# ugadiarov-la-phystech-edu/OCRL

Measured on AMD Instinct MI355X. Metric: images/sec (node) SLATE pretrain 128x128, 6 slots, 3 iters, higher is better.
Workload: dtype f32

## Files before the change

ocrl_amd/csrc/attention.hip:

```cpp
#include "common.h"
#include "kernels.h"
#include <stdlib.h>

#define FA_BLK 64
#ifndef FA_LPT
#define FA_LPT 1
#endif
#ifndef FA_BWD_WGS
#define FA_BWD_WGS 3
#endif

typedef float f32x4_t __attribute__((ext_vector_type(4)));

template <int DH>
struct FaCfg {
    static constexpr int NC = DH / 16;
    static constexpr int LD = DH + 4;
};

template <int DH>
__device__ inline void fa_load_tile(float* s, const float* __restrict__ g, long long bt0, int row0, int T, int d, int hoff, float scale) {
    constexpr int F4 = DH / 4;
    constexpr int LD = FaCfg<DH>::LD;
    for (int idx = threadIdx.x; idx < FA_BLK * F4; idx += 256) {
        const int c4 = idx % F4, r = idx / F4;
        float4 v = make_float4(0.f, 0.f, 0.f, 0.f);
        if (row0 + r < T) v = *reinterpret_cast<const float4*>(g + (bt0 + row0 + r) * d + hoff + c4 * 4);
        v.x *= scale; v.y *= scale; v.z *= scale; v.w *= scale;
        *reinterpret_cast<float4*>(s + r * LD + c4 * 4) = v;
    }
}

template <int DH> struct FaRegs { static constexpr int N = (FA_BLK * (DH / 4) + 255) / 256; };
template <int DH>
__device__ inline void fa_fetch(float4 (&r)[FaRegs<DH>::N], const float* __restrict__ g, long long bt0, int row0, int T, int d, int hoff) {
    constexpr int F4 = DH / 4;
#pragma unroll
    for (int i = 0; i < FaRegs<DH>::N; ++i) {
        const int idx = threadIdx.x + i * 256;
        const int c4 = idx % F4, row = idx / F4;
        r[i] = make_float4(0.f, 0.f, 0.f, 0.f);
        if (idx < FA_BLK * F4 && row0 + row < T) r[i] = *reinterpret_cast<const float4*>(g + (bt0 + row0 + row) * d + hoff + c4 * 4);
    }
}
template <int DH>
__device__ inline void fa_commit(float* s, const float4 (&r)[FaRegs<DH>::N], float scale) {
    constexpr int F4 = DH / 4, LD = FaCfg<DH>::LD;
#pragma unroll
    for (int i = 0; i < FaRegs<DH>::N; ++i) {
        const int idx = threadIdx.x + i * 256;
        if (idx < FA_BLK * F4) *reinterpret_cast<float4*>(s + (idx / F4) * LD + (idx % F4) * 4) = make_float4(r[i].x * scale, r[i].y * scale, r[i].z * scale, r[i].w * scale);
    }
}

__device__ inline int fa_block_index(int j, long long bh, int nblk) {
    const long long rot = nblk >= 8 ? bh : bh / (8 / (nblk > 0 ? nblk : 1) > 0 ? 8 / nblk : 1);
    return (int)((j + rot) % nblk);
}

#define MFMA16(a, b, c) __builtin_amdgcn_mfma_f32_16x16x4f32((a), (b), (c), 0, 0, 0)

template <int DH>
__global__ __launch_bounds__(256, 4) void attn_fwd_kernel(AttnArgs p) {
    constexpr int NC = FaCfg<DH>::NC, LD = FaCfg<DH>::LD;
    __shared__ __attribute__((aligned(16))) float Ks[FA_BLK * LD];
    __shared__ __attribute__((aligned(16))) float Vs[FA_BLK * LD];
    const int nqb = (p.T + FA_BLK - 1) / FA_BLK;
    int bid = blockIdx.x;
    const int nbh = gridDim.x / nqb;
    const int qb = FA_LPT ? nqb - 1 - bid / nbh : fa_block_index(bid % nqb, bid / nqb, nqb);
    bid = FA_LPT ? bid % nbh : bid / nqb;
    const int hd = bid % p.h;
    const long long b = bid / p.h;
    const int T = p.T, d = p.ld, hoff = hd * DH;
    const long long bt0 = b * T;
    const int lane = threadIdx.x & 63, wv = threadIdx.x >> 6;
    const int li = lane & 15, g = lane >> 4;
    const int q_abs = qb * FA_BLK + wv * 16 + li;
    const float scale = rsqrtf((float)DH);
    const long long bh = b * p.h + hd;

    float4 qf[NC];
#pragma unroll
    for (int c = 0; c < NC; ++c) {
        float4 v = make_float4(0.f, 0.f, 0.f, 0.f);
        if (q_abs < T) v = *reinterpret_cast<const float4*>(p.q + (bt0 + q_abs) * d + hoff + 16 * c + 4 * g);
        qf[c] = make_float4(v.x * scale, v.y * scale, v.z * scale, v.w * scale);
    }
    f32x4_t o[NC];
#pragma unroll
    for (int c = 0; c < NC; ++c) o[c] = (f32x4_t){0.f, 0.f, 0.f, 0.f};
    float m = -INFINITY, l = 0.f;
    const uint32_t thr = drop_thresh(p.p);
    const float dsc = p.p > 0.f ? 1.0f / (1.0f - p.p) : 1.f;

    float4 rk[FaRegs<DH>::N], rv[FaRegs<DH>::N];
    fa_fetch<DH>(rk, p.k, bt0, 0, T, d, hoff);
    fa_fetch<DH>(rv, p.v, bt0, 0, T, d, hoff);
    for (int kt = 0; kt <= qb; ++kt) {
        __syncthreads();
        fa_commit<DH>(Ks, rk, 1.f);
        fa_commit<DH>(Vs, rv, 1.f);
        __syncthreads();
        if (kt < qb) {
            fa_fetch<DH>(rk, p.k, bt0, (kt + 1) * FA_BLK, T, d, hoff);
            fa_fetch<DH>(rv, p.v, bt0, (kt + 1) * FA_BLK, T, d, hoff);
        }
        f32x4_t s[4];
#pragma unroll
        for (int st = 0; st < 4; ++st) s[st] = (f32x4_t){0.f, 0.f, 0.f, 0.f};
#pragma unroll
        for (int c = 0; c < NC; ++c) {
            float4 a[4];
#pragma unroll
            for (int st = 0; st < 4; ++st) a[st] = *reinterpret_cast<const float4*>(Ks + (16 * st + li) * LD + 16 * c + 4 * g);
#pragma unroll
            for (int st = 0; st < 4; ++st) s[st] = MFMA16(a[st].x, qf[c].x, s[st]);
#pragma unroll
            for (int st = 0; st < 4; ++st) s[st] = MFMA16(a[st].y, qf[c].y, s[st]);
#pragma unroll
            for (int st = 0; st < 4; ++st) s[st] = MFMA16(a[st].z, qf[c].z, s[st]);
#pragma unroll
            for (int st = 0; st < 4; ++st) s[st] = MFMA16(a[st].w, qf[c].w, s[st]);
        }
        float mx = -INFINITY;
        if (kt == qb || (kt + 1) * FA_BLK > T) {
#pragma unroll
            for (int st = 0; st < 4; ++st) {
                const int key0 = kt * FA_BLK + 16 * st + 4 * g;
#pragma unroll
                for (int r = 0; r < 4; ++r)
                    if (key0 + r > q_abs || key0 + r >= T) s[st][r] = -INFINITY;
            }
        }
#pragma unroll
        for (int st = 0; st < 4; ++st)
#pragma unroll
            for (int r = 0; r < 4; ++r) mx = fmaxf(mx, s[st][r]);
        mx = fmaxf(mx, __shfl_xor(mx, 16, 64));
        mx = fmaxf(mx, __shfl_xor(mx, 32, 64));
        const float m_new = fmaxf(m, mx);
        const float alpha = (m_new == -INFINITY) ? 1.f : __expf(m - m_new);
        float rs = 0.f;
#pragma unroll
        for (int st = 0; st < 4; ++st)
#pragma unroll
            for (int r = 0; r < 4; ++r) {
                const float e = (m_new == -INFINITY) ? 0.f : __expf(s[st][r] - m_new);
                s[st][r] = e;
                rs += e;
            }
        rs += __shfl_xor(rs, 16, 64);
        rs += __shfl_xor(rs, 32, 64);
        l = l * alpha + rs;
        m = m_new;
#pragma unroll
        for (int c = 0; c < NC; ++c) o[c] *= alpha;
        if (p.p > 0.f) {
#pragma unroll
            for (int st = 0; st < 4; ++st) {
                const uint64_t idx = ((uint64_t)bh * T + (uint64_t)(q_abs < T ? q_abs : 0)) * T + (uint64_t)(kt * FA_BLK + 16 * st + 4 * g);
                const uint2 bits = rng_bits4(p.seed, p.site, idx >> 2);
#pragma unroll
                for (int r = 0; r < 4; ++r) s[st][r] = rng_keep(bits, r, thr) ? s[st][r] * dsc : 0.f;
            }
        }
        float av[2][4][NC];
#pragma unroll
        for (int r = 0; r < 4; ++r)
#pragma unroll
            for (int c = 0; c < NC; ++c) av[0][r][c] = Vs[(4 * g + r) * LD + 16 * c + li];
#pragma unroll
        for (int st = 0; st < 4; ++st) {
            if (st + 1 < 4) {
#pragma unroll
                for (int r = 0; r < 4; ++r)
#pragma unroll
                    for (int c = 0; c < NC; ++c) av[(st + 1) & 1][r][c] = Vs[(16 * (st + 1) + 4 * g + r) * LD + 16 * c + li];
            }
            __builtin_amdgcn_sched_barrier(0);
#pragma unroll
            for (int r = 0; r < 4; ++r)
#pragma unroll
                for (int c = 0; c < NC; ++c) o[c] = MFMA16(av[st & 1][r][c], s[st][r], o[c]);
            __builtin_amdgcn_sched_barrier(0);
        }
    }
    if (q_abs < T) {
        const float inv = 1.0f / l;
#pragma unroll
        for (int c = 0; c < NC; ++c)
            *reinterpret_cast<float4*>(p.o + (bt0 + q_abs) * p.d + hoff + 16 * c + 4 * g) = make_float4(o[c][0] * inv, o[c][1] * inv, o[c][2] * inv, o[c][3] * inv);
        if (g == 0) p.lse[bh * T + q_abs] = m + __logf(l);
    }
}

__global__ __launch_bounds__(256) void attn_delta_kernel(const float* __restrict__ dO, const float* __restrict__ O, float* __restrict__ delta, long long BT, int T, int d,
                                                         int h) {
    __shared__ float part[256];
    const int F4 = d >> 2, RPB = 256 / F4, HF = F4 / h;
    const int rl = threadIdx.x / F4, c4 = threadIdx.x - rl * F4;
    const long long row = (long long)blockIdx.x * RPB + rl;
    float s = 0.f;
    if (rl < RPB && row < BT) {
        const float4 x = *reinterpret_cast<const float4*>(dO + row * d + c4 * 4), y = *reinterpret_cast<const float4*>(O + row * d + c4 * 4);
        s = x.x * y.x + x.y * y.y + x.z * y.z + x.w * y.w;
    }
    part[threadIdx.x] = s;
    __syncthreads();
    if ((int)threadIdx.x < RPB * h) {
        const int r2 = threadIdx.x / h, hd = threadIdx.x - r2 * h;
        const long long row2 = (long long)blockIdx.x * RPB + r2;
        if (row2 < BT) {
            float t = 0.f;
            for (int k = 0; k < HF; ++k) t += part[r2 * F4 + hd * HF + k];
            const long long bb = row2 / T, q = row2 % T;
            delta[(bb * h + hd) * T + q] = t;
        }
    }
}

template <int DH>
__global__ __launch_bounds__(256, FA_BWD_WGS) void attn_bwd_kv_kernel(AttnArgs p) {
    constexpr int NC = FaCfg<DH>::NC, LD = FaCfg<DH>::LD;
    __shared__ __attribute__((aligned(16))) float Qs[FA_BLK * LD];
    __shared__ __attribute__((aligned(16))) float Gs[FA_BLK * LD];
    __shared__ float Ls[FA_BLK], Ds[FA_BLK];
    const int nkb = (p.T + FA_BLK - 1) / FA_BLK;
    int bid = blockIdx.x;
    const int nbh = gridDim.x / nkb;
    const int kb = FA_LPT ? bid / nbh : fa_block_index(bid % nkb, bid / nkb, nkb);
    bid = FA_LPT ? bid % nbh : bid / nkb;
    const int hd = bid % p.h;
    const long long b = bid / p.h;
    const int T = p.T, d = p.ld, hoff = hd * DH;
    const long long bt0 = b * T;
    const int lane = threadIdx.x & 63, wv = threadIdx.x >> 6;
    const int li = lane & 15, g = lane >> 4;
    const int k_abs = kb * FA_BLK + wv * 16 + li;
    const float scale = rsqrtf((float)DH);
    const long long bh = b * p.h + hd;

    float4 kf[NC], vf[NC];
#pragma unroll
    for (int c = 0; c < NC; ++c) {
        kf[c] = make_float4(0.f, 0.f, 0.f, 0.f);
        vf[c] = kf[c];
        if (k_abs < T) {
            kf[c] = *reinterpret_cast<const float4*>(p.k + (bt0 + k_abs) * d + hoff + 16 * c + 4 * g);
            vf[c] = *reinterpret_cast<const float4*>(p.v + (bt0 + k_abs) * d + hoff + 16 * c + 4 * g);
        }
    }
    f32x4_t dk[NC], dv[NC];
#pragma unroll
    for (int c = 0; c < NC; ++c) { dk[c] = (f32x4_t){0.f, 0.f, 0.f, 0.f}; dv[c] = dk[c]; }
    const uint32_t thr = drop_thresh(p.p);
    const float dsc = p.p > 0.f ? 1.0f / (1.0f - p.p) : 1.f;

    float4 rq[FaRegs<DH>::N], rg[FaRegs<DH>::N];
    float rl = 0.f, rd = 0.f;
    auto fetch = [&](int qt) {
        fa_fetch<DH>(rq, p.q, bt0, qt * FA_BLK, T, d, hoff);
        fa_fetch<DH>(rg, p.dO, bt0, qt * FA_BLK, T, p.d, hoff);
        if (threadIdx.x < FA_BLK) {
            const int qq = qt * FA_BLK + threadIdx.x;
            rl = qq < T ? p.lse[bh * T + qq] : 0.f;
            rd = qq < T ? p.delta[bh * T + qq] : 0.f;
        }
    };
    fetch(kb);
    for (int qt = kb; qt < nkb; ++qt) {
        __syncthreads();
        fa_commit<DH>(Qs, rq, scale);
        fa_commit<DH>(Gs, rg, 1.f);
        if (threadIdx.x < FA_BLK) { Ls[threadIdx.x] = rl; Ds[threadIdx.x] = rd; }
        __syncthreads();
        if (qt + 1 < nkb) fetch(qt + 1);
#pragma unroll
        for (int sq = 0; sq < 4; ++sq) {
            f32x4_t s = (f32x4_t){0.f, 0.f, 0.f, 0.f}, dp = s;
#pragma unroll
            for (int c = 0; c < NC; ++c) {
                const float4 a = *reinterpret_cast<const float4*>(Qs + (16 * sq + li) * LD + 16 * c + 4 * g);
                s = MFMA16(a.x, kf[c].x, s);
                s = MFMA16(a.y, kf[c].y, s);
                s = MFMA16(a.z, kf[c].z, s);
                s = MFMA16(a.w, kf[c].w, s);
                const float4 e = *reinterpret_cast<const float4*>(Gs + (16 * sq + li) * LD + 16 * c + 4 * g);
                dp = MFMA16(e.x, vf[c].x, dp);
                dp = MFMA16(e.y, vf[c].y, dp);
                dp = MFMA16(e.z, vf[c].z, dp);
                dp = MFMA16(e.w, vf[c].w, dp);
            }
            uint2 hb = make_uint2(0u, 0u);
            if (p.p > 0.f) {
                const int qh = qt * FA_BLK + 16 * sq + 4 * g + (li & 3);
                const uint64_t idx = ((uint64_t)bh * T + (uint64_t)(qh < T ? qh : 0)) * T + (uint64_t)(k_abs < T ? k_abs : 0);
                hb = rng_bits4(p.seed, p.site, idx >> 2);
            }
            uint2 hq[4];
            hq[0] = make_uint2(__builtin_amdgcn_update_dpp(0, (int)hb.x, 0x00, 0xF, 0xF, false), __builtin_amdgcn_update_dpp(0, (int)hb.y, 0x00, 0xF, 0xF, false));
            hq[1] = make_uint2(__builtin_amdgcn_update_dpp(0, (int)hb.x, 0x55, 0xF, 0xF, false), __builtin_amdgcn_update_dpp(0, (int)hb.y, 0x55, 0xF, 0xF, false));
            hq[2] = make_uint2(__builtin_amdgcn_update_dpp(0, (int)hb.x, 0xAA, 0xF, 0xF, false), __builtin_amdgcn_update_dpp(0, (int)hb.y, 0xAA, 0xF, 0xF, false));
            hq[3] = make_uint2(__builtin_amdgcn_update_dpp(0, (int)hb.x, 0xFF, 0xF, 0xF, false), __builtin_amdgcn_update_dpp(0, (int)hb.y, 0xFF, 0xF, 0xF, false));
            f32x4_t pd, ds;
#pragma unroll
            for (int r = 0; r < 4; ++r) {
                const int ql = 16 * sq + 4 * g + r;
                const int qa = qt * FA_BLK + ql;
                float pr = 0.f;
                if (qa < T && k_abs <= qa && k_abs < T) pr = __expf(s[r] - Ls[ql]);
                float keep = 1.f;
                if (p.p > 0.f) keep = rng_keep(hq[r], li & 3, thr) ? dsc : 0.f;
                pd[r] = pr * keep;
                ds[r] = pr * (dp[r] * keep - Ds[ql]);
            }
            float ag[4][NC], aq[4][NC];
#pragma unroll
            for (int r = 0; r < 4; ++r)
#pragma unroll
                for (int c = 0; c < NC; ++c) {
                    ag[r][c] = Gs[(16 * sq + 4 * g + r) * LD + 16 * c + li];
                    aq[r][c] = Qs[(16 * sq + 4 * g + r) * LD + 16 * c + li];
                }
            __builtin_amdgcn_sched_barrier(0);
#pragma unroll
            for (int r = 0; r < 4; ++r)
#pragma unroll
                for (int c = 0; c < NC; ++c) {
                    dv[c] = MFMA16(ag[r][c], pd[r], dv[c]);
                    dk[c] = MFMA16(aq[r][c], ds[r], dk[c]);
                }
        }
    }
    if (k_abs < T) {
#pragma unroll
        for (int c = 0; c < NC; ++c) {
            *reinterpret_cast<float4*>(p.dv + (bt0 + k_abs) * d + hoff + 16 * c + 4 * g) = make_float4(dv[c][0], dv[c][1], dv[c][2], dv[c][3]);
            *reinterpret_cast<float4*>(p.dk + (bt0 + k_abs) * d + hoff + 16 * c + 4 * g) = make_float4(dk[c][0], dk[c][1], dk[c][2], dk[c][3]);
        }
    }
}

template <int DH>
__global__ __launch_bounds__(256, FA_BWD_WGS) void attn_bwd_q_kernel(AttnArgs p) {
    constexpr int NC = FaCfg<DH>::NC, LD = FaCfg<DH>::LD;
    __shared__ __attribute__((aligned(16))) float Ks[FA_BLK * LD];
    __shared__ __attribute__((aligned(16))) float Vs[FA_BLK * LD];
    const int nqb = (p.T + FA_BLK - 1) / FA_BLK;
    int bid = blockIdx.x;
    const int nbh = gridDim.x / nqb;
    const int qb = FA_LPT ? nqb - 1 - bid / nbh : fa_block_index(bid % nqb, bid / nqb, nqb);
    bid = FA_LPT ? bid % nbh : bid / nqb;
    const int hd = bid % p.h;
    const long long b = bid / p.h;
    const int T = p.T, d = p.ld, hoff = hd * DH;
    const long long bt0 = b * T;
    const int lane = threadIdx.x & 63, wv = threadIdx.x >> 6;
    const int li = lane & 15, g = lane >> 4;
    const int q_abs = qb * FA_BLK + wv * 16 + li;
    const float scale = rsqrtf((float)DH);
    const long long bh = b * p.h + hd;

    float4 qf[NC], gf[NC];
#pragma unroll
    for (int c = 0; c < NC; ++c) {
        qf[c] = make_float4(0.f, 0.f, 0.f, 0.f);
        gf[c] = qf[c];
        if (q_abs < T) {
            const float4 v = *reinterpret_cast<const float4*>(p.q + (bt0 + q_abs) * d + hoff + 16 * c + 4 * g);
            qf[c] = make_float4(v.x * scale, v.y * scale, v.z * scale, v.w * scale);
            gf[c] = *reinterpret_cast<const float4*>(p.dO + (bt0 + q_abs) * p.d + hoff + 16 * c + 4 * g);
        }
    }
    const float lse = q_abs < T ? p.lse[bh * T + q_abs] : 0.f;
    const float dlt = q_abs < T ? p.delta[bh * T + q_abs] : 0.f;
    f32x4_t dq[NC];
#pragma unroll
    for (int c = 0; c < NC; ++c) dq[c] = (f32x4_t){0.f, 0.f, 0.f, 0.f};
    const uint32_t thr = drop_thresh(p.p);
    const float dsc = p.p > 0.f ? 1.0f / (1.0f - p.p) : 1.f;

    float4 rk[FaRegs<DH>::N], rv[FaRegs<DH>::N];
    fa_fetch<DH>(rk, p.k, bt0, 0, T, d, hoff);
    fa_fetch<DH>(rv, p.v, bt0, 0, T, d, hoff);
    for (int kt = 0; kt <= qb; ++kt) {
        __syncthreads();
        fa_commit<DH>(Ks, rk, 1.f);
        fa_commit<DH>(Vs, rv, 1.f);
        __syncthreads();
        if (kt < qb) {
            fa_fetch<DH>(rk, p.k, bt0, (kt + 1) * FA_BLK, T, d, hoff);
            fa_fetch<DH>(rv, p.v, bt0, (kt + 1) * FA_BLK, T, d, hoff);
        }
        f32x4_t sS[4], sP[4];
#pragma unroll
        for (int st = 0; st < 4; ++st) { sS[st] = (f32x4_t){0.f, 0.f, 0.f, 0.f}; sP[st] = sS[st]; }
#pragma unroll
        for (int c = 0; c < NC; ++c) {
            float4 a[4], e[4];
#pragma unroll
            for (int st = 0; st < 4; ++st) {
                a[st] = *reinterpret_cast<const float4*>(Ks + (16 * st + li) * LD + 16 * c + 4 * g);
                e[st] = *reinterpret_cast<const float4*>(Vs + (16 * st + li) * LD + 16 * c + 4 * g);
            }
#pragma unroll
            for (int st = 0; st < 4; ++st) { sS[st] = MFMA16(a[st].x, qf[c].x, sS[st]); sP[st] = MFMA16(e[st].x, gf[c].x, sP[st]); }
#pragma unroll
            for (int st = 0; st < 4; ++st) { sS[st] = MFMA16(a[st].y, qf[c].y, sS[st]); sP[st] = MFMA16(e[st].y, gf[c].y, sP[st]); }
#pragma unroll
            for (int st = 0; st < 4; ++st) { sS[st] = MFMA16(a[st].z, qf[c].z, sS[st]); sP[st] = MFMA16(e[st].z, gf[c].z, sP[st]); }
#pragma unroll
            for (int st = 0; st < 4; ++st) { sS[st] = MFMA16(a[st].w, qf[c].w, sS[st]); sP[st] = MFMA16(e[st].w, gf[c].w, sP[st]); }
        }
#pragma unroll
        for (int st = 0; st < 4; ++st) {
            const int key0 = kt * FA_BLK + 16 * st + 4 * g;
            uint2 bits = make_uint2(0u, 0u);
            if (p.p > 0.f) {
                const uint64_t idx = ((uint64_t)bh * T + (uint64_t)(q_abs < T ? q_abs : 0)) * T + (uint64_t)key0;
                bits = rng_bits4(p.seed, p.site, idx >> 2);
            }
#pragma unroll
            for (int r = 0; r < 4; ++r) {
                float pr = 0.f;
                if (q_abs < T && key0 + r <= q_abs && key0 + r < T) pr = __expf(sS[st][r] - lse);
                float keep = 1.f;
                if (p.p > 0.f) keep = rng_keep(bits, r, thr) ? dsc : 0.f;
                sS[st][r] = pr * (sP[st][r] * keep - dlt);
            }
        }
        float ak[2][4][NC];
#pragma unroll
        for (int r = 0; r < 4; ++r)
#pragma unroll
            for (int c = 0; c < NC; ++c) ak[0][r][c] = Ks[(4 * g + r) * LD + 16 * c + li];
#pragma unroll
        for (int st = 0; st < 4; ++st) {
            if (st + 1 < 4) {
#pragma unroll
                for (int r = 0; r < 4; ++r)
#pragma unroll
                    for (int c = 0; c < NC; ++c) ak[(st + 1) & 1][r][c] = Ks[(16 * (st + 1) + 4 * g + r) * LD + 16 * c + li];
            }
            __builtin_amdgcn_sched_barrier(0);
#pragma unroll
            for (int r = 0; r < 4; ++r)
#pragma unroll
                for (int c = 0; c < NC; ++c) dq[c] = MFMA16(ak[st & 1][r][c], sS[st][r], dq[c]);
            __builtin_amdgcn_sched_barrier(0);
        }
    }
    if (q_abs < T) {
#pragma unroll
        for (int c = 0; c < NC; ++c)
            *reinterpret_cast<float4*>(p.dq + (bt0 + q_abs) * d + hoff + 16 * c + 4 * g) =
                make_float4(dq[c][0] * scale, dq[c][1] * scale, dq[c][2] * scale, dq[c][3] * scale);
    }
}

#define FB_KB 128
template <int DH>
__global__ __launch_bounds__(512, 2) void attn_bwd_fused_kernel(AttnArgs p) {
    constexpr int NC = FaCfg<DH>::NC, LD = FaCfg<DH>::LD, SLD = FB_KB + 4;
    __shared__ __attribute__((aligned(16))) float Qs[FA_BLK * LD];
    __shared__ __attribute__((aligned(16))) float Gs[FA_BLK * LD];
    __shared__ __attribute__((aligned(16))) float Ss[FA_BLK * SLD];
    __shared__ __attribute__((aligned(16))) float Rs[4 * 16 * DH];
    __shared__ float Ls[FA_BLK], Ds[FA_BLK];
    const int hd = blockIdx.x % p.h;
    const long long b = blockIdx.x / p.h;
    const int T = p.T, d = p.ld, hoff = hd * DH;
    const long long bt0 = b * T;
    const int tid = threadIdx.x, lane = tid & 63, wv = tid >> 6;
    const int li = lane & 15, g = lane >> 4;
    const int qs = wv & 3, kh = wv >> 2;
    const float scale = rsqrtf((float)DH);
    const long long bh = b * p.h + hd;
    const uint32_t thr = drop_thresh(p.p);
    const float dsc = p.p > 0.f ? 1.0f / (1.0f - p.p) : 1.f;
    const int nqt = (T + FA_BLK - 1) / FA_BLK, nkb = (T + FB_KB - 1) / FB_KB;
    constexpr int F4 = DH / 4;
#pragma unroll 1
    for (int kb = 0; kb < nkb; ++kb) {
        const int k_abs = kb * FB_KB + wv * 16 + li;
        float4 kf[NC], vf[NC];
#pragma unroll
        for (int c = 0; c < NC; ++c) {
            kf[c] = make_float4(0.f, 0.f, 0.f, 0.f);
            vf[c] = kf[c];
            if (k_abs < T) {
                kf[c] = *reinterpret_cast<const float4*>(p.k + (bt0 + k_abs) * d + hoff + 16 * c + 4 * g);
                vf[c] = *reinterpret_cast<const float4*>(p.v + (bt0 + k_abs) * d + hoff + 16 * c + 4 * g);
            }
        }
        float kq[16][NC];
#pragma unroll
        for (int s = 0; s < 16; ++s) {
            const int key = kb * FB_KB + kh * 64 + 16 * (s >> 2) + 4 * g + (s & 3);
#pragma unroll
            for (int c = 0; c < NC; ++c) kq[s][c] = key < T ? p.k[(bt0 + key) * d + hoff + 16 * c + li] * scale : 0.f;
        }
        f32x4_t dk[NC], dv[NC];
#pragma unroll
        for (int c = 0; c < NC; ++c) { dk[c] = (f32x4_t){0.f, 0.f, 0.f, 0.f}; dv[c] = dk[c]; }
#pragma unroll 1
        for (int qt = (kb * FB_KB) / FA_BLK; qt < nqt; ++qt) {
            __syncthreads();
            for (int idx = tid; idx < FA_BLK * F4; idx += 512) {
                const int c4 = idx % F4, r = idx / F4;
                float4 q4 = make_float4(0.f, 0.f, 0.f, 0.f), g4 = q4;
                if (qt * FA_BLK + r < T) {
                    q4 = *reinterpret_cast<const float4*>(p.q + (bt0 + qt * FA_BLK + r) * d + hoff + c4 * 4);
                    g4 = *reinterpret_cast<const float4*>(p.dO + (bt0 + qt * FA_BLK + r) * p.d + hoff + c4 * 4);
                }
                *reinterpret_cast<float4*>(Qs + r * LD + c4 * 4) = make_float4(q4.x * scale, q4.y * scale, q4.z * scale, q4.w * scale);
                *reinterpret_cast<float4*>(Gs + r * LD + c4 * 4) = g4;
            }
            if (tid < FA_BLK) {
                const int qq = qt * FA_BLK + tid;
                Ls[tid] = qq < T ? p.lse[bh * T + qq] : 0.f;
                Ds[tid] = qq < T ? p.delta[bh * T + qq] : 0.f;
            }
            __syncthreads();
#pragma unroll
            for (int sq = 0; sq < 4; ++sq) {
                f32x4_t s = (f32x4_t){0.f, 0.f, 0.f, 0.f}, dp = s;
#pragma unroll
                for (int c = 0; c < NC; ++c) {
                    const float4 a = *reinterpret_cast<const float4*>(Qs + (16 * sq + li) * LD + 16 * c + 4 * g);
                    s = MFMA16(a.x, kf[c].x, s);
                    s = MFMA16(a.y, kf[c].y, s);
                    s = MFMA16(a.z, kf[c].z, s);
                    s = MFMA16(a.w, kf[c].w, s);
                    const float4 e = *reinterpret_cast<const float4*>(Gs + (16 * sq + li) * LD + 16 * c + 4 * g);
                    dp = MFMA16(e.x, vf[c].x, dp);
                    dp = MFMA16(e.y, vf[c].y, dp);
                    dp = MFMA16(e.z, vf[c].z, dp);
                    dp = MFMA16(e.w, vf[c].w, dp);
                }
                uint2 hb = make_uint2(0u, 0u);
                if (p.p > 0.f) {
                    const int qh = qt * FA_BLK + 16 * sq + 4 * g + (li & 3);
                    const uint64_t idx = ((uint64_t)bh * T + (uint64_t)(qh < T ? qh : 0)) * T + (uint64_t)(k_abs < T ? k_abs : 0);
                    hb = rng_bits4(p.seed, p.site, idx >> 2);
                }
                uint2 hq[4];
                hq[0] = make_uint2(__builtin_amdgcn_update_dpp(0, (int)hb.x, 0x00, 0xF, 0xF, false), __builtin_amdgcn_update_dpp(0, (int)hb.y, 0x00, 0xF, 0xF, false));
                hq[1] = make_uint2(__builtin_amdgcn_update_dpp(0, (int)hb.x, 0x55, 0xF, 0xF, false), __builtin_amdgcn_update_dpp(0, (int)hb.y, 0x55, 0xF, 0xF, false));
                hq[2] = make_uint2(__builtin_amdgcn_update_dpp(0, (int)hb.x, 0xAA, 0xF, 0xF, false), __builtin_amdgcn_update_dpp(0, (int)hb.y, 0xAA, 0xF, 0xF, false));
                hq[3] = make_uint2(__builtin_amdgcn_update_dpp(0, (int)hb.x, 0xFF, 0xF, 0xF, false), __builtin_amdgcn_update_dpp(0, (int)hb.y, 0xFF, 0xF, 0xF, false));
                f32x4_t pd, ds;
#pragma unroll
                for (int r = 0; r < 4; ++r) {
                    const int ql = 16 * sq + 4 * g + r;
                    const int qa = qt * FA_BLK + ql;
                    float pr = 0.f;
                    if (qa < T && k_abs <= qa && k_abs < T) pr = __expf(s[r] - Ls[ql]);
                    float keep = 1.f;
                    if (p.p > 0.f) keep = rng_keep(hq[r], li & 3, thr) ? dsc : 0.f;
                    pd[r] = pr * keep;
                    ds[r] = pr * (dp[r] * keep - Ds[ql]);
                    Ss[ql * SLD + wv * 16 + li] = ds[r];
                }
                float ag[4][NC], aq[4][NC];
#pragma unroll
                for (int r = 0; r < 4; ++r)
#pragma unroll
                    for (int c = 0; c < NC; ++c) {
                        ag[r][c] = Gs[(16 * sq + 4 * g + r) * LD + 16 * c + li];
                        aq[r][c] = Qs[(16 * sq + 4 * g + r) * LD + 16 * c + li];
                    }
                __builtin_amdgcn_sched_barrier(0);
#pragma unroll
                for (int r = 0; r < 4; ++r)
#pragma unroll
                    for (int c = 0; c < NC; ++c) {
                        dv[c] = MFMA16(ag[r][c], pd[r], dv[c]);
                        dk[c] = MFMA16(aq[r][c], ds[r], dk[c]);
                    }
            }
            __syncthreads();
            f32x4_t dq[NC];
#pragma unroll
            for (int c = 0; c < NC; ++c) dq[c] = (f32x4_t){0.f, 0.f, 0.f, 0.f};
#pragma unroll
            for (int j = 0; j < 4; ++j) {
                const float4 a4 = *reinterpret_cast<const float4*>(Ss + (16 * qs + li) * SLD + kh * 64 + 16 * j + 4 * g);
#pragma unroll
                for (int c = 0; c < NC; ++c) {
                    dq[c] = MFMA16(a4.x, kq[4 * j + 0][c], dq[c]);
                    dq[c] = MFMA16(a4.y, kq[4 * j + 1][c], dq[c]);
                    dq[c] = MFMA16(a4.z, kq[4 * j + 2][c], dq[c]);
                    dq[c] = MFMA16(a4.w, kq[4 * j + 3][c], dq[c]);
                }
            }
            if (kh == 1) {
#pragma unroll
                for (int c = 0; c < NC; ++c)
#pragma unroll
                    for (int r = 0; r < 4; ++r) Rs[(qs * 16 + 4 * g + r) * DH + 16 * c + li] = dq[c][r];
            }
            __syncthreads();
            if (kh == 0) {
                const bool first = kb == 0;
#pragma unroll
                for (int r = 0; r < 4; ++r) {
                    const int qa = qt * FA_BLK + 16 * qs + 4 * g + r;
                    if (qa >= T) continue;
                    float* dst = p.dq + (bt0 + qa) * d + hoff + li;
#pragma unroll
                    for (int c = 0; c < NC; ++c) {
                        const float v = dq[c][r] + Rs[(qs * 16 + 4 * g + r) * DH + 16 * c + li];
                        dst[16 * c] = first ? v : dst[16 * c] + v;
                    }
                }
            }
        }
        if (k_abs < T) {
#pragma unroll
            for (int c = 0; c < NC; ++c) {
                *reinterpret_cast<float4*>(p.dv + (bt0 + k_abs) * d + hoff + 16 * c + 4 * g) = make_float4(dv[c][0], dv[c][1], dv[c][2], dv[c][3]);
                *reinterpret_cast<float4*>(p.dk + (bt0 + k_abs) * d + hoff + 16 * c + 4 * g) = make_float4(dk[c][0], dk[c][1], dk[c][2], dk[c][3]);
            }
        }
    }
}

template <int DH>
static int attn_launch_dh(const AttnArgs& a, int mode, hipStream_t st) {
    const int nblk = cdiv(a.T, FA_BLK);
    const dim3 grid(a.B * a.h * nblk), blk(256);
    if (mode == 0) {
        hipLaunchKernelGGL((attn_fwd_kernel<DH>), grid, blk, 0, st, a);
        OCRL_CHECK_LAUNCH("attn_fwd");
    } else {
        const long long BT = (long long)a.B * a.T;
        OCRL_REQUIRE(a.d % 4 == 0 && a.d <= 1024 && (a.d / 4) % a.h == 0, "attention: d must be a multiple of 4*h, <= 1024");
        hipLaunchKernelGGL(attn_delta_kernel, dim3(cdiv(BT, 256 / (a.d / 4))), dim3(256), 0, st, a.dO, a.o, a.delta, BT, a.T, a.d, a.h);
        OCRL_CHECK_LAUNCH("attn_delta");
        const char* fe = getenv("OCRL_ATTN_BWD");
        if (fe && atoi(fe) == 1) {
            hipLaunchKernelGGL((attn_bwd_fused_kernel<DH>), dim3(a.B * a.h), dim3(512), 0, st, a);
            OCRL_CHECK_LAUNCH("attn_bwd_fused");
        } else {
        hipLaunchKernelGGL((attn_bwd_kv_kernel<DH>), grid, blk, 0, st, a);
        OCRL_CHECK_LAUNCH("attn_bwd_kv");
        hipLaunchKernelGGL((attn_bwd_q_kernel<DH>), grid, blk, 0, st, a);
        OCRL_CHECK_LAUNCH("attn_bwd_q");
        }
    }
    return 0;
}

int attn_launch(const AttnArgs& a, int mode, hipStream_t st) {
    OCRL_REQUIRE(a.B > 0 && a.T > 0 && a.h > 0 && a.d % a.h == 0 && a.ld >= a.d && a.ld % 4 == 0, "attention: bad shape");
    OCRL_REQUIRE(a.q && a.k && a.v && a.o && a.lse, "attention: missing buffers");
    if (mode) OCRL_REQUIRE(a.dO && a.dq && a.dk && a.dv && a.delta, "attention backward: missing buffers");
    OCRL_REQUIRE((long long)a.T * a.T * a.B * a.h < (1ll << 62), "attention: too large");
    const int pi = prof_begin(mode ? PROF_ATTN_BWD : PROF_ATTN_FWD, st);
    int rc;
    switch (a.d / a.h) {
        case 16: rc = attn_launch_dh<16>(a, mode, st); break;
        case 32: rc = attn_launch_dh<32>(a, mode, st); break;
        case 48: rc = attn_launch_dh<48>(a, mode, st); break;
        case 64: rc = attn_launch_dh<64>(a, mode, st); break;
        default: ocrl_set_error("attention: head dim %d unsupported (16/32/48/64)", a.d / a.h); return 1;
    }
    prof_end(pi, st);
    return rc;
}
```

Measured before the change: 1700.

## Add 128-row tiled attention backward kernels as default for head dims up to 48

Adds new dK/dV and dQ backward kernels where each wave owns 32 rows instead of 16, so a block covers 128 keys or queries. Each Q/dO or K/V tile staged in shared memory is reused across twice as many rows, cutting global traffic and per-tile overhead. These kernels become the default path (OCRL_ATTN_BWD unset) for DH<=48, while DH 64 keeps the old kernels. The cost is more registers per thread and half as many blocks, which may reduce occupancy and parallelism for short sequences.

```diff
diff --git a/ocrl_amd/csrc/attention.hip b/ocrl_amd/csrc/attention.hip
--- a/ocrl_amd/csrc/attention.hip
+++ b/ocrl_amd/csrc/attention.hip
@@ -456,6 +456,279 @@
         for (int c = 0; c < NC; ++c)
             *reinterpret_cast<float4*>(p.dq + (bt0 + q_abs) * d + hoff + 16 * c + 4 * g) =
                 make_float4(dq[c][0] * scale, dq[c][1] * scale, dq[c][2] * scale, dq[c][3] * scale);
+    }
+}
+
+#define FB2_BLK 128
+#ifndef FB2_WGS
+#define FB2_WGS 2
+#endif
+template <int DH>
+__global__ __launch_bounds__(256, FB2_WGS) void attn_bwd_kv128_kernel(AttnArgs p) {
+    constexpr int NC = FaCfg<DH>::NC, LD = FaCfg<DH>::LD;
+    __shared__ __attribute__((aligned(16))) float Qs[FA_BLK * LD];
+    __shared__ __attribute__((aligned(16))) float Gs[FA_BLK * LD];
+    __shared__ float Ls[FA_BLK], Ds[FA_BLK];
+    const int nkb = (p.T + FB2_BLK - 1) / FB2_BLK, nqt = (p.T + FA_BLK - 1) / FA_BLK;
+    int bid = blockIdx.x;
+    const int nbh = gridDim.x / nkb;
+    const int kb = FA_LPT ? bid / nbh : fa_block_index(bid % nkb, bid / nkb, nkb);
+    bid = FA_LPT ? bid % nbh : bid / nkb;
+    const int hd = bid % p.h;
+    const long long b = bid / p.h;
+    const int T = p.T, d = p.ld, hoff = hd * DH;
+    const long long bt0 = b * T;
+    const int lane = threadIdx.x & 63, wv = threadIdx.x >> 6;
+    const int li = lane & 15, g = lane >> 4;
+    const int k0 = kb * FB2_BLK + wv * 32;
+    int ka[2];
+    ka[0] = k0 + li;
+    ka[1] = k0 + 16 + li;
+    const float scale = rsqrtf((float)DH);
+    const long long bh = b * p.h + hd;
+
+    float4 kf[2][NC], vf[2][NC];
+#pragma unroll
+    for (int j = 0; j < 2; ++j)
+#pragma unroll
+        for (int c = 0; c < NC; ++c) {
+            kf[j][c] = make_float4(0.f, 0.f, 0.f, 0.f);
+            vf[j][c] = kf[j][c];
+            if (ka[j] < T) {
+                kf[j][c] = *reinterpret_cast<const float4*>(p.k + (bt0 + ka[j]) * d + hoff + 16 * c + 4 * g);
+                vf[j][c] = *reinterpret_cast<const float4*>(p.v + (bt0 + ka[j]) * d + hoff + 16 * c + 4 * g);
+            }
+        }
+    f32x4_t dk[2][NC], dv[2][NC];
+#pragma unroll
+    for (int j = 0; j < 2; ++j)
+#pragma unroll
+        for (int c = 0; c < NC; ++c) { dk[j][c] = (f32x4_t){0.f, 0.f, 0.f, 0.f}; dv[j][c] = dk[j][c]; }
+    const uint32_t thr = drop_thresh(p.p);
+    const float dsc = p.p > 0.f ? 1.0f / (1.0f - p.p) : 1.f;
+
+    float4 rq[FaRegs<DH>::N], rg[FaRegs<DH>::N];
+    float rl = 0.f, rd = 0.f;
+    auto fetch = [&](int qt) {
+        fa_fetch<DH>(rq, p.q, bt0, qt * FA_BLK, T, d, hoff);
+        fa_fetch<DH>(rg, p.dO, bt0, qt * FA_BLK, T, p.d, hoff);
+        if (threadIdx.x < FA_BLK) {
+            const int qq = qt * FA_BLK + threadIdx.x;
+            rl = qq < T ? p.lse[bh * T + qq] : 0.f;
+            rd = qq < T ? p.delta[bh * T + qq] : 0.f;
+        }
+    };
+    const int qt0 = kb * (FB2_BLK / FA_BLK);
+    fetch(qt0);
+    for (int qt = qt0; qt < nqt; ++qt) {
+        __syncthreads();
+        fa_commit<DH>(Qs, rq, scale);
+        fa_commit<DH>(Gs, rg, 1.f);
+        if (threadIdx.x < FA_BLK) { Ls[threadIdx.x] = rl; Ds[threadIdx.x] = rd; }
+        __syncthreads();
+        if (qt + 1 < nqt) fetch(qt + 1);
+#pragma unroll 1
+        for (int sq = 0; sq < 4; ++sq) {
+            if (qt * FA_BLK + 16 * sq + 15 < k0) continue;
+            f32x4_t s[2], dp[2];
+#pragma unroll
+            for (int j = 0; j < 2; ++j) { s[j] = (f32x4_t){0.f, 0.f, 0.f, 0.f}; dp[j] = s[j]; }
+#pragma unroll
+            for (int c = 0; c < NC; ++c) {
+                const float4 a = *reinterpret_cast<const float4*>(Qs + (16 * sq + li) * LD + 16 * c + 4 * g);
+                const float4 e = *reinterpret_cast<const float4*>(Gs + (16 * sq + li) * LD + 16 * c + 4 * g);
+#pragma unroll
+                for (int j = 0; j < 2; ++j) { s[j] = MFMA16(a.x, kf[j][c].x, s[j]); dp[j] = MFMA16(e.x, vf[j][c].x, dp[j]); }
+#pragma unroll
+                for (int j = 0; j < 2; ++j) { s[j] = MFMA16(a.y, kf[j][c].y, s[j]); dp[j] = MFMA16(e.y, vf[j][c].y, dp[j]); }
+#pragma unroll
+                for (int j = 0; j < 2; ++j) { s[j] = MFMA16(a.z, kf[j][c].z, s[j]); dp[j] = MFMA16(e.z, vf[j][c].z, dp[j]); }
+#pragma unroll
+                for (int j = 0; j < 2; ++j) { s[j] = MFMA16(a.w, kf[j][c].w, s[j]); dp[j] = MFMA16(e.w, vf[j][c].w, dp[j]); }
+            }
+            float ag[4][NC], aq[4][NC];
+#pragma unroll
+            for (int r = 0; r < 4; ++r)
+#pragma unroll
+                for (int c = 0; c < NC; ++c) {
+                    ag[r][c] = Gs[(16 * sq + 4 * g + r) * LD + 16 * c + li];
+                    aq[r][c] = Qs[(16 * sq + 4 * g + r) * LD + 16 * c + li];
+                }
+            float lq[4], dl[4];
+#pragma unroll
+            for (int r = 0; r < 4; ++r) { lq[r] = Ls[16 * sq + 4 * g + r]; dl[r] = Ds[16 * sq + 4 * g + r]; }
+#pragma unroll
+            for (int j = 0; j < 2; ++j) {
+                uint2 hb = make_uint2(0u, 0u);
+                if (p.p > 0.f) {
+                    const int qh = qt * FA_BLK + 16 * sq + 4 * g + (li & 3);
+                    const uint64_t idx = ((uint64_t)bh * T + (uint64_t)(qh < T ? qh : 0)) * T + (uint64_t)(ka[j] < T ? ka[j] : 0);
+                    hb = rng_bits4(p.seed, p.site, idx >> 2);
+                }
+                uint2 hq[4];
+                hq[0] = make_uint2(__builtin_amdgcn_update_dpp(0, (int)hb.x, 0x00, 0xF, 0xF, false), __builtin_amdgcn_update_dpp(0, (int)hb.y, 0x00, 0xF, 0xF, false));
+                hq[1] = make_uint2(__builtin_amdgcn_update_dpp(0, (int)hb.x, 0x55, 0xF, 0xF, false), __builtin_amdgcn_update_dpp(0, (int)hb.y, 0x55, 0xF, 0xF, false));
+                hq[2] = make_uint2(__builtin_amdgcn_update_dpp(0, (int)hb.x, 0xAA, 0xF, 0xF, false), __builtin_amdgcn_update_dpp(0, (int)hb.y, 0xAA, 0xF, 0xF, false));
+                hq[3] = make_uint2(__builtin_amdgcn_update_dpp(0, (int)hb.x, 0xFF, 0xF, 0xF, false), __builtin_amdgcn_update_dpp(0, (int)hb.y, 0xFF, 0xF, 0xF, false));
+#pragma unroll
+                for (int r = 0; r < 4; ++r) {
+                    const int qa = qt * FA_BLK + 16 * sq + 4 * g + r;
+                    float pr = 0.f;
+                    if (qa < T && ka[j] <= qa && ka[j] < T) pr = __expf(s[j][r] - lq[r]);
+                    float keep = 1.f;
+                    if (p.p > 0.f) keep = rng_keep(hq[r], li & 3, thr) ? dsc : 0.f;
+                    s[j][r] = pr * keep;
+                    dp[j][r] = pr * (dp[j][r] * keep - dl[r]);
+                }
+            }
+            __builtin_amdgcn_sched_barrier(0);
+#pragma unroll
+            for (int r = 0; r < 4; ++r)
+#pragma unroll
+                for (int c = 0; c < NC; ++c)
+#pragma unroll
+                    for (int j = 0; j < 2; ++j) {
+                        dv[j][c] = MFMA16(ag[r][c], s[j][r], dv[j][c]);
+                        dk[j][c] = MFMA16(aq[r][c], dp[j][r], dk[j][c]);
+                    }
+        }
+    }
+#pragma unroll
+    for (int j = 0; j < 2; ++j) {
+        if (ka[j] < T) {
+#pragma unroll
+            for (int c = 0; c < NC; ++c) {
+                *reinterpret_cast<float4*>(p.dv + (bt0 + ka[j]) * d + hoff + 16 * c + 4 * g) = make_float4(dv[j][c][0], dv[j][c][1], dv[j][c][2], dv[j][c][3]);
+                *reinterpret_cast<float4*>(p.dk + (bt0 + ka[j]) * d + hoff + 16 * c + 4 * g) = make_float4(dk[j][c][0], dk[j][c][1], dk[j][c][2], dk[j][c][3]);
+            }
+        }
+    }
+}
+
+template <int DH>
+__global__ __launch_bounds__(256, FB2_WGS) void attn_bwd_q128_kernel(AttnArgs p) {
+    constexpr int NC = FaCfg<DH>::NC, LD = FaCfg<DH>::LD;
+    __shared__ __attribute__((aligned(16))) float Ks[FA_BLK * LD];
+    __shared__ __attribute__((aligned(16))) float Vs[FA_BLK * LD];
+    const int nqb = (p.T + FB2_BLK - 1) / FB2_BLK;
+    int bid = blockIdx.x;
+    const int nbh = gridDim.x / nqb;
+    const int qb = FA_LPT ? nqb - 1 - bid / nbh : fa_block_index(bid % nqb, bid / nqb, nqb);
+    bid = FA_LPT ? bid % nbh : bid / nqb;
+    const int hd = bid % p.h;
+    const long long b = bid / p.h;
+    const int T = p.T, d = p.ld, hoff = hd * DH;
+    const long long bt0 = b * T;
+    const int lane = threadIdx.x & 63, wv = threadIdx.x >> 6;
+    const int li = lane & 15, g = lane >> 4;
+    const int q0 = qb * FB2_BLK + wv * 32;
+    int qa[2];
+    qa[0] = q0 + li;
+    qa[1] = q0 + 16 + li;
+    const float scale = rsqrtf((float)DH);
+    const long long bh = b * p.h + hd;
+
+    float4 qf[2][NC], gf[2][NC];
+    float lse[2], dlt[2];
+#pragma unroll
+    for (int j = 0; j < 2; ++j) {
+#pragma unroll
+        for (int c = 0; c < NC; ++c) {
+            qf[j][c] = make_float4(0.f, 0.f, 0.f, 0.f);
+            gf[j][c] = qf[j][c];
+            if (qa[j] < T) {
+                const float4 v = *reinterpret_cast<const float4*>(p.q + (bt0 + qa[j]) * d + hoff + 16 * c + 4 * g);
+                qf[j][c] = make_float4(v.x * scale, v.y * scale, v.z * scale, v.w * scale);
+                gf[j][c] = *reinterpret_cast<const float4*>(p.dO + (bt0 + qa[j]) * p.d + hoff + 16 * c + 4 * g);
+            }
+        }
+        lse[j] = qa[j] < T ? p.lse[bh * T + qa[j]] : 0.f;
+        dlt[j] = qa[j] < T ? p.delta[bh * T + qa[j]] : 0.f;
+    }
+    f32x4_t dq[2][NC];
+#pragma unroll
+    for (int j = 0; j < 2; ++j)
+#pragma unroll
+        for (int c = 0; c < NC; ++c) dq[j][c] = (f32x4_t){0.f, 0.f, 0.f, 0.f};
+    const uint32_t thr = drop_thresh(p.p);
+    const float dsc = p.p > 0.f ? 1.0f / (1.0f - p.p) : 1.f;
+
+    const int nkt = min(T - 1, qb * FB2_BLK + FB2_BLK - 1) / FA_BLK + 1;
+    float4 rk[FaRegs<DH>::N], rv[FaRegs<DH>::N];
+    fa_fetch<DH>(rk, p.k, bt0, 0, T, d, hoff);
+    fa_fetch<DH>(rv, p.v, bt0, 0, T, d, hoff);
+    for (int kt = 0; kt < nkt; ++kt) {
+        __syncthreads();
+        fa_commit<DH>(Ks, rk, 1.f);
+        fa_commit<DH>(Vs, rv, 1.f);
+        __syncthreads();
+        if (kt + 1 < nkt) {
+            fa_fetch<DH>(rk, p.k, bt0, (kt + 1) * FA_BLK, T, d, hoff);
+            fa_fetch<DH>(rv, p.v, bt0, (kt + 1) * FA_BLK, T, d, hoff);
+        }
+#pragma unroll 1
+        for (int st = 0; st < 4; ++st) {
+            const int key0 = kt * FA_BLK + 16 * st;
+            if (key0 > q0 + 31) continue;
+            float4 a[NC], e[NC];
+            float ak[4][NC];
+#pragma unroll
+            for (int c = 0; c < NC; ++c) {
+                a[c] = *reinterpret_cast<const float4*>(Ks + (16 * st + li) * LD + 16 * c + 4 * g);
+                e[c] = *reinterpret_cast<const float4*>(Vs + (16 * st + li) * LD + 16 * c + 4 * g);
+            }
+#pragma unroll
+            for (int r = 0; r < 4; ++r)
+#pragma unroll
+                for (int c = 0; c < NC; ++c) ak[r][c] = Ks[(16 * st + 4 * g + r) * LD + 16 * c + li];
+            f32x4_t sS[2], sP[2];
+#pragma unroll
+            for (int j = 0; j < 2; ++j) { sS[j] = (f32x4_t){0.f, 0.f, 0.f, 0.f}; sP[j] = sS[j]; }
+#pragma unroll
+            for (int c = 0; c < NC; ++c) {
+#pragma unroll
+                for (int j = 0; j < 2; ++j) { sS[j] = MFMA16(a[c].x, qf[j][c].x, sS[j]); sP[j] = MFMA16(e[c].x, gf[j][c].x, sP[j]); }
+#pragma unroll
+                for (int j = 0; j < 2; ++j) { sS[j] = MFMA16(a[c].y, qf[j][c].y, sS[j]); sP[j] = MFMA16(e[c].y, gf[j][c].y, sP[j]); }
+#pragma unroll
+                for (int j = 0; j < 2; ++j) { sS[j] = MFMA16(a[c].z, qf[j][c].z, sS[j]); sP[j] = MFMA16(e[c].z, gf[j][c].z, sP[j]); }
+#pragma unroll
+                for (int j = 0; j < 2; ++j) { sS[j] = MFMA16(a[c].w, qf[j][c].w, sS[j]); sP[j] = MFMA16(e[c].w, gf[j][c].w, sP[j]); }
+            }
+            const int kg = key0 + 4 * g;
+#pragma unroll
+            for (int j = 0; j < 2; ++j) {
+                uint2 bits = make_uint2(0u, 0u);
+                if (p.p > 0.f) {
+                    const uint64_t idx = ((uint64_t)bh * T + (uint64_t)(qa[j] < T ? qa[j] : 0)) * T + (uint64_t)kg;
+                    bits = rng_bits4(p.seed, p.site, idx >> 2);
+                }
+#pragma unroll
+                for (int r = 0; r < 4; ++r) {
+                    float pr = 0.f;
+                    if (qa[j] < T && kg + r <= qa[j] && kg + r < T) pr = __expf(sS[j][r] - lse[j]);
+                    float keep = 1.f;
+                    if (p.p > 0.f) keep = rng_keep(bits, r, thr) ? dsc : 0.f;
+                    sS[j][r] = pr * (sP[j][r] * keep - dlt[j]);
+                }
+            }
+            __builtin_amdgcn_sched_barrier(0);
+#pragma unroll
+            for (int r = 0; r < 4; ++r)
+#pragma unroll
+                for (int c = 0; c < NC; ++c)
+#pragma unroll
+                    for (int j = 0; j < 2; ++j) dq[j][c] = MFMA16(ak[r][c], sS[j][r], dq[j][c]);
+        }
+    }
+#pragma unroll
+    for (int j = 0; j < 2; ++j) {
+        if (qa[j] < T) {
+#pragma unroll
+            for (int c = 0; c < NC; ++c)
+                *reinterpret_cast<float4*>(p.dq + (bt0 + qa[j]) * d + hoff + 16 * c + 4 * g) =
+                    make_float4(dq[j][c][0] * scale, dq[j][c][1] * scale, dq[j][c][2] * scale, dq[j][c][3] * scale);
+        }
     }
 }
 
@@ -640,14 +913,21 @@
         hipLaunchKernelGGL(attn_delta_kernel, dim3(cdiv(BT, 256 / (a.d / 4))), dim3(256), 0, st, a.dO, a.o, a.delta, BT, a.T, a.d, a.h);
         OCRL_CHECK_LAUNCH("attn_delta");
         const char* fe = getenv("OCRL_ATTN_BWD");
-        if (fe && atoi(fe) == 1) {
+        const int form = fe ? atoi(fe) : 3;
+        if (form == 1) {
             hipLaunchKernelGGL((attn_bwd_fused_kernel<DH>), dim3(a.B * a.h), dim3(512), 0, st, a);
             OCRL_CHECK_LAUNCH("attn_bwd_fused");
-        } else {
-        hipLaunchKernelGGL((attn_bwd_kv_kernel<DH>), grid, blk, 0, st, a);
-        OCRL_CHECK_LAUNCH("attn_bwd_kv");
-        hipLaunchKernelGGL((attn_bwd_q_kernel<DH>), grid, blk, 0, st, a);
-        OCRL_CHECK_LAUNCH("attn_bwd_q");
+        } else if (form == 2 || DH > 48) {
+            hipLaunchKernelGGL((attn_bwd_kv_kernel<DH>), grid, blk, 0, st, a);
+            OCRL_CHECK_LAUNCH("attn_bwd_kv");
+            hipLaunchKernelGGL((attn_bwd_q_kernel<DH>), grid, blk, 0, st, a);
+            OCRL_CHECK_LAUNCH("attn_bwd_q");
+        } else if constexpr (DH <= 48) {
+            const dim3 grid2(a.B * a.h * cdiv(a.T, FB2_BLK));
+            hipLaunchKernelGGL((attn_bwd_kv128_kernel<DH>), grid2, blk, 0, st, a);
+            OCRL_CHECK_LAUNCH("attn_bwd_kv128");
+            hipLaunchKernelGGL((attn_bwd_q128_kernel<DH>), grid2, blk, 0, st, a);
+            OCRL_CHECK_LAUNCH("attn_bwd_q128");
         }
     }
     return 0;
```

Result: no change. 1710 (median of 6 runs) (+0.6%).
